# GATB/bcalm

Measured on AMD Instinct MI355X. Metric: distinct k-mers/s reads->unitigs k=31, higher is better.
Workload: dtype u64; 1 GPU; BASELINE config 3: synthetic 100000000 x 150 bp reads per GPU, k=31, abundance-min 2, 1% substitutions, 30x coverage; multi_gpu=single GPU, minimizer_size=16, log2_partitions=22

## Files before the change

bcalm_amd/csrc/devrt.h:

```cpp
#pragma once
#include <stdint.h>

#ifdef CDBG_HOSTSIM
#include "hostsim.h"
#else
#include <hip/hip_runtime.h>
#define CDBG_HD __host__ __device__ __forceinline__
#define CDBG_DEV __device__ __forceinline__
#define CDBG_SPIN_YIELD() __builtin_amdgcn_s_sleep(1)
#define CDBG_LAUNCH(kern, grid, block, stream, ...) \
    hipLaunchKernelGGL(kern, dim3((unsigned)(grid)), dim3((unsigned)(block)), 0, stream, __VA_ARGS__)
#define CDBG_SHARED __shared__
#define CDBG_WAVE_SYNC() __builtin_amdgcn_wave_barrier()
#define CDBG_PIN64(x) asm volatile("" : "+v"(x))
#endif

namespace cdbg {

CDBG_DEV uint64_t atomic_add_u64(uint64_t* p, uint64_t v) {
    return (uint64_t)atomicAdd((unsigned long long*)p, (unsigned long long)v);
}
CDBG_DEV uint64_t atomic_cas_u64(uint64_t* p, uint64_t cmp, uint64_t v) {
    return (uint64_t)atomicCAS((unsigned long long*)p, (unsigned long long)cmp, (unsigned long long)v);
}
CDBG_DEV uint64_t atomic_exch_u64(uint64_t* p, uint64_t v) {
    return (uint64_t)atomicExch((unsigned long long*)p, (unsigned long long)v);
}
#define CDBG_COMPILER_BARRIER() asm volatile("" ::: "memory")
CDBG_DEV uint64_t ld_agent_u64(const uint64_t* p) {
#ifdef CDBG_HOSTSIM
    return *p;
#else
    return __hip_atomic_load(p, __ATOMIC_RELAXED, __HIP_MEMORY_SCOPE_AGENT);
#endif
}
CDBG_DEV uint32_t ld_volatile_u32(const uint32_t* p) { return *(const volatile uint32_t*)p; }
CDBG_DEV uint32_t atomic_add_u32(uint32_t* p, uint32_t v) { return atomicAdd(p, v); }
CDBG_DEV uint32_t atomic_sub_u32(uint32_t* p, uint32_t v) { return atomicSub(p, v); }
CDBG_DEV uint32_t atomic_or_u32(uint32_t* p, uint32_t v) { return atomicOr(p, v); }
CDBG_DEV uint32_t atomic_cas_u32(uint32_t* p, uint32_t cmp, uint32_t v) { return atomicCAS(p, cmp, v); }
CDBG_DEV uint32_t atomic_max_u32(uint32_t* p, uint32_t v) { return atomicMax(p, v); }
CDBG_DEV uint32_t atomic_min_u32(uint32_t* p, uint32_t v) { return atomicMin(p, v); }
CDBG_DEV void atomic_or_u64(uint64_t* p, uint64_t v) { (void)atomicOr((unsigned long long*)p, (unsigned long long)v); }
CDBG_DEV uint64_t ld_unaligned_u64(const uint8_t* p) { uint64_t v; __builtin_memcpy(&v, p, 8); return v; }
CDBG_DEV void st_unaligned_u64(uint8_t* p, uint64_t v) { __builtin_memcpy(p, &v, 8); }
CDBG_DEV void st_unaligned_u32(uint8_t* p, uint32_t v) { __builtin_memcpy(p, &v, 4); }
CDBG_DEV void st_unaligned_u16(uint8_t* p, uint16_t v) { __builtin_memcpy(p, &v, 2); }

#ifdef CDBG_HOSTSIM
CDBG_DEV uint32_t wave_incl_sum_u32(uint32_t v) {
    const int lane = (int)(threadIdx.x & 63);
    for (int d = 1; d < 64; d <<= 1) { const uint32_t x = __shfl_up(v, (unsigned)d); if (lane >= d) v += x; }
    return v;
}
CDBG_DEV uint32_t wave_readlane_u32(uint32_t v, int src_lane) { return __shfl(v, src_lane); }
CDBG_DEV uint32_t alignbit_u32(uint32_t hi, uint32_t lo, uint32_t sh) { return (uint32_t)((((uint64_t)hi << 32) | lo) >> (sh & 31u)); }
#else
CDBG_DEV uint32_t wave_incl_sum_u32(uint32_t v) {
    v += (uint32_t)__builtin_amdgcn_update_dpp(0, (int)v, 0x111, 0xf, 0xf, false);
    v += (uint32_t)__builtin_amdgcn_update_dpp(0, (int)v, 0x112, 0xf, 0xf, false);
    v += (uint32_t)__builtin_amdgcn_update_dpp(0, (int)v, 0x114, 0xf, 0xf, false);
    v += (uint32_t)__builtin_amdgcn_update_dpp(0, (int)v, 0x118, 0xf, 0xf, false);
    v += (uint32_t)__builtin_amdgcn_update_dpp(0, (int)v, 0x142, 0xa, 0xf, false);
    v += (uint32_t)__builtin_amdgcn_update_dpp(0, (int)v, 0x143, 0xc, 0xf, false);
    return v;
}
CDBG_DEV uint32_t wave_readlane_u32(uint32_t v, int src_lane) { return (uint32_t)__builtin_amdgcn_readlane((int)v, src_lane); }
CDBG_DEV uint32_t alignbit_u32(uint32_t hi, uint32_t lo, uint32_t sh) { return __builtin_amdgcn_alignbit(hi, lo, sh); }
#endif
#ifdef CDBG_HOSTSIM
CDBG_DEV uint32_t uni_u32(uint32_t v) { return __shfl(v, 0); }
#define CDBG_NOINLINE
#define CDBG_DEV_NOINL inline
#define CDBG_LDS_BARRIER() __syncthreads()
#define CDBG_LDS_FENCE() do { } while (0)
#else
CDBG_DEV uint32_t uni_u32(uint32_t v) { return (uint32_t)__builtin_amdgcn_readfirstlane((int)v); }
#define CDBG_NOINLINE __attribute__((noinline))
#define CDBG_DEV_NOINL __device__
#define CDBG_LDS_BARRIER() do { __builtin_amdgcn_fence(__ATOMIC_RELEASE, "workgroup", "local"); __builtin_amdgcn_s_barrier(); \
                                __builtin_amdgcn_fence(__ATOMIC_ACQUIRE, "workgroup", "local"); } while (0)
#define CDBG_LDS_FENCE() __builtin_amdgcn_fence(__ATOMIC_RELEASE, "workgroup", "local")
#endif
CDBG_DEV uint64_t uni_u64(uint64_t v) { return ((uint64_t)uni_u32((uint32_t)(v >> 32)) << 32) | uni_u32((uint32_t)v); }
#ifdef CDBG_HOSTSIM
CDBG_DEV uint32_t wave_append_slots(uint32_t* cursor) { return atomic_add_u32(cursor, 1u); }
#else
CDBG_DEV uint32_t wave_append_slots(uint32_t* cursor) {
    const uint64_t act = __ballot(1);
    const uint32_t rank = __builtin_amdgcn_mbcnt_hi((uint32_t)(act >> 32), __builtin_amdgcn_mbcnt_lo((uint32_t)act, 0u));
    uint32_t base = 0;
    if (rank == 0) base = atomic_add_u32(cursor, (uint32_t)__popcll(act));
    return uni_u32(base) + rank;
}
#endif
#ifdef CDBG_HOSTSIM
CDBG_DEV uint32_t lane_pick_u32(uint64_t mask, uint32_t v, int lane) { return ((mask >> lane) & 1ULL) ? v : 0u; }
#else
CDBG_DEV uint32_t lane_pick_u32(uint64_t mask, uint32_t v, int) {
    uint32_t r;
    asm("v_cndmask_b32_e64 %0, 0, %1, %2" : "=v"(r) : "v"(v), "s"(mask));
    return r;
}
#endif
CDBG_DEV uint64_t wave_sum_u64(uint64_t v) {
#pragma unroll
    for (int d = 32; d >= 1; d >>= 1) v += __shfl_xor(v, d);
    return v;
}

}
```

bcalm_amd/csrc/k_scan.h:

```cpp
#pragma once
#include "kmer.h"

namespace cdbg {

#if defined(CDBG_PROFILE_PHASES) && !defined(CDBG_HOSTSIM)
#define CDBG_SPH(i) do { if (threadIdx.x == 0) { const uint64_t t_ = wall_clock64(); sph[i] += t_ - st_prev; st_prev = t_; } } while (0)
#else
#define CDBG_SPH(i) do { } while (0)
#endif
constexpr int SCAN_THREADS = 256;
constexpr int SCAN_GRID = 256 * 2;
constexpr int SCAN_TILE = 4096;
constexpr int SCAN_PKW = (SCAN_TILE + 16 + 256) / 16 + 11;
static_assert(SCAN_PKW % 2 == 0, "validity halves must fill whole 32-bit words");
constexpr int SCAN_NKEY = SCAN_TILE + 256;

template <int W> struct RecFmt {
    static constexpr int RW = 2 * W;
    static constexpr int CAPB = 32 * RW - 8;
};

struct ScanParams {
    const uint8_t* reads;
    uint64_t nbytes;
    uint64_t nbytes_padded;
    int k, m, log_np;
    int rank_bits, rank;
    uint32_t* part_count;
    uint64_t* part_cursor;
    uint64_t* records;
    uint64_t* stats;
    uint64_t n_tiles;
    uint32_t tile_stride, tile_offset;
    uint32_t part_cap; uint32_t* part_fill;
    uint64_t* spill_recs; uint32_t* spill_part; uint64_t* spill_cursor; uint64_t spill_cap; uint32_t* error;
    uint32_t emit_all, npl;
    const uint64_t* var_limit;
    const uint64_t* ovf;
    const uint64_t* part_off;
    uint32_t defer_slices, defer_shift, defer_nseg, defer_seg_cap;
    uint64_t defer_map;
    uint64_t* defer_recs; uint32_t* defer_part; uint32_t* defer_count;
};
constexpr int SCAN_DEFER_MAX = 16;
constexpr int SCAN_HIST = 0, SCAN_EMIT = 1, SCAN_EMIT_CAPPED = 2;
constexpr int OVF_CAP_BITS = 28;
constexpr uint64_t OVF_CAP_MASK = (1ULL << OVF_CAP_BITS) - 1ULL;

CDBG_DEV uint64_t scan_get64(const uint32_t* pk, int bitoff) {
    const int w = bitoff >> 5, sh = bitoff & 31;
    uint64_t x = ((uint64_t)pk[w] << 32) | pk[w + 1];
    return sh ? ((x << sh) | ((uint64_t)pk[w + 2] >> (32 - sh))) : x;
}
CDBG_DEV bool scan_all_valid(const uint32_t* vm, int q, int len) {
    while (len > 0) {
        const int w = q >> 5, sh = q & 31;
        uint64_t x = ((uint64_t)vm[w + 1] << 32) | vm[w];
        uint32_t bits = (uint32_t)(x >> sh);
        const int c = len < 32 ? len : 32;
        const uint32_t msk = c == 32 ? 0xFFFFFFFFu : ((1u << c) - 1u);
        if ((bits & msk) != msk) return false;
        q += c; len -= c;
    }
    return true;
}

struct alignas(16) RecPair { uint64_t lo, hi; };
#ifndef CDBG_REC16_W1
#define CDBG_REC16_W1 0
#endif
template <int MODE>
CDBG_DEV uint32_t scan_reserve_record(const ScanParams& P, uint32_t lpart) {
    if (MODE == SCAN_HIST) { atomic_add_u32(&P.part_count[lpart], 1u); return 0u; }
    return atomic_add_u32(&P.part_fill[lpart], 1u);
}
template <int W, int MODE>
CDBG_DEV uint64_t* scan_record_dst(const ScanParams& P, uint32_t lpart, uint32_t j) {
    constexpr int RW = RecFmt<W>::RW;
    if (MODE == SCAN_HIST) return nullptr;
    uint64_t* dst;
    bool fits;
    if (MODE == SCAN_EMIT) {
        uint64_t pos = (uint64_t)j;
        fits = true;
        if (P.part_off != nullptr) {
            pos += P.part_off[lpart];
            fits = P.var_limit == nullptr || pos < P.var_limit[lpart];
        }
        dst = P.records + pos * RW;
    } else {
        fits = j < P.part_cap;
        dst = P.records + ((uint64_t)lpart * P.part_cap + j) * RW;
        if (!fits && P.ovf != nullptr) {
            const uint64_t d = P.ovf[lpart];
            if ((uint64_t)j < (d & OVF_CAP_MASK)) { fits = true; dst = P.records + ((d >> OVF_CAP_BITS) + j) * RW; }
        }
    }
    if (!fits) {
        const uint64_t o = atomic_add_u64(P.spill_cursor, 1ULL);
        if (o >= P.spill_cap) { *P.error = 6; return nullptr; }
        P.spill_part[o] = lpart;
        dst = P.spill_recs + o * RW;
    }
    return dst;
}
template <int W>
CDBG_DEV void scan_store_words(uint64_t* dst, const uint64_t (&w)[RecFmt<W>::RW]) {
    constexpr int RW = RecFmt<W>::RW;
    static_assert(RW % 2 == 0, "records are pairs of words");
    if (RW == 2 && !CDBG_REC16_W1) {
        dst[1] = w[1]; CDBG_COMPILER_BARRIER(); dst[0] = w[0];
        return;
    }
#pragma unroll
    for (int i = RW - 2; i >= 0; i -= 2) {
        RecPair v; v.lo = w[i]; v.hi = w[i + 1];
        *reinterpret_cast<RecPair*>(&dst[i]) = v;
    }
}
template <int W>
CDBG_DEV void scan_record_words(const uint32_t* pk, int bitoff, uint32_t meta, uint64_t (&w)[RecFmt<W>::RW]) {
    constexpr int RW = RecFmt<W>::RW;
#pragma unroll
    for (int wv = 0; wv < RW; ++wv) {
        uint64_t x = scan_get64(pk, bitoff + 64 * wv);
        if (wv == RW - 1) x = (x & ~0xFFFFULL) | meta;
        w[RW - 1 - wv] = x;
    }
}
template <int W, int MODE>
CDBG_DEV void scan_finish_record(const ScanParams& P, const uint32_t* pk, int bitoff, uint32_t meta, uint32_t lpart, uint32_t j) {
    constexpr int RW = RecFmt<W>::RW;
    if (MODE == SCAN_HIST) return;
    uint64_t* dst = scan_record_dst<W, MODE>(P, lpart, j);
    if (dst == nullptr) return;
    if (RW == 2 && !CDBG_REC16_W1) {
#pragma unroll
        for (int wv = 0; wv < RW; ++wv) {
            uint64_t x = scan_get64(pk, bitoff + 64 * wv);
            if (wv == RW - 1) x = (x & ~0xFFFFULL) | meta;
            dst[RW - 1 - wv] = x;
        }
        return;
    }
#pragma unroll
    for (int wv = 0; wv < RW; wv += 2) {
        const uint64_t hi = scan_get64(pk, bitoff + 64 * wv);
        uint64_t lo = scan_get64(pk, bitoff + 64 * (wv + 1));
        if (wv + 1 == RW - 1) lo = (lo & ~0xFFFFULL) | meta;
        RecPair v; v.lo = lo; v.hi = hi;
        *reinterpret_cast<RecPair*>(&dst[RW - 2 - wv]) = v;
    }
}
template <int W, int MODE>
CDBG_DEV void scan_emit_record(const ScanParams& P, const uint32_t* pk, int bitoff, uint32_t meta, uint32_t lpart, uint32_t* sdefer) {
    if (MODE == SCAN_EMIT_CAPPED && P.defer_slices > 1u) {
        const uint32_t sl = (uint32_t)(P.defer_map >> (4u * (lpart >> P.defer_shift))) & 15u;
        if (sl) {
            constexpr int RW = RecFmt<W>::RW;
            uint32_t slot = P.defer_seg_cap;
            for (uint32_t q = 1; q < P.defer_slices; ++q)
                if (sl == q) slot = wave_append_slots(&sdefer[q]);
            if (slot < P.defer_seg_cap) {
                const uint64_t at = ((uint64_t)(sl - 1u) * P.defer_nseg + blockIdx.x) * P.defer_seg_cap + slot;
                uint64_t w[RW];
                scan_record_words<W>(pk, bitoff, meta, w);
                uint64_t* dst = P.defer_recs + at * RW;
#pragma unroll
                for (int i = 0; i < RW; i += 2) { RecPair v; v.lo = w[i]; v.hi = w[i + 1]; *reinterpret_cast<RecPair*>(&dst[i]) = v; }
                P.defer_part[at] = lpart;
                return;
            }
        }
    }
    scan_finish_record<W, MODE>(P, pk, bitoff, meta, lpart, scan_reserve_record<MODE>(P, lpart));
}
template <int MODE>
CDBG_DEV void scan_defer_init(const ScanParams& P, uint32_t* sdefer) { if (MODE == SCAN_EMIT_CAPPED && P.defer_slices > 1u && threadIdx.x < (unsigned)SCAN_DEFER_MAX) sdefer[threadIdx.x] = 0; }
template <int MODE>
CDBG_DEV void scan_defer_publish(const ScanParams& P, const uint32_t* sdefer) {
    if (MODE == SCAN_EMIT_CAPPED && P.defer_slices > 1u && threadIdx.x >= 1u && threadIdx.x < P.defer_slices)
        P.defer_count[(uint64_t)(threadIdx.x - 1u) * P.defer_nseg + blockIdx.x] = sdefer[threadIdx.x];
}

struct PlaceParams { ScanParams sp; uint32_t slice; };
template <int W>
__global__ void __launch_bounds__(64) k_place(PlaceParams Q) {
    constexpr int RW = RecFmt<W>::RW;
    constexpr int PLACE_U = RW <= 2 ? 4 : RW <= 4 ? 2 : 1;
    const ScanParams& P = Q.sp;
    for (uint32_t seg = blockIdx.x; seg < P.defer_nseg; seg += gridDim.x) {
        const uint64_t sidx = (uint64_t)(Q.slice - 1u) * P.defer_nseg + seg;
        const uint32_t n0 = uni_u32(P.defer_count[sidx]);
        const uint32_t n = n0 < P.defer_seg_cap ? n0 : P.defer_seg_cap;
        const uint64_t base = sidx * P.defer_seg_cap;
        for (uint32_t b = 0; b < n; b += 64u * PLACE_U) {
            uint64_t w[PLACE_U][RW]; uint32_t p[PLACE_U], j[PLACE_U];
#pragma unroll
            for (int u = 0; u < PLACE_U; ++u) {
                const uint32_t i = b + (uint32_t)u * 64u + threadIdx.x;
                p[u] = 0xFFFFFFFFu;
                if (i < n) {
                    p[u] = P.defer_part[base + i];
                    const uint64_t* src = P.defer_recs + (base + i) * RW;
#pragma unroll
                    for (int q = 0; q < RW; q += 2) { const RecPair v = *reinterpret_cast<const RecPair*>(&src[q]); w[u][q] = v.lo; w[u][q + 1] = v.hi; }
                }
            }
#pragma unroll
            for (int u = 0; u < PLACE_U; ++u) if (p[u] != 0xFFFFFFFFu) j[u] = scan_reserve_record<SCAN_EMIT_CAPPED>(P, p[u]);
#pragma unroll
            for (int u = 0; u < PLACE_U; ++u) if (p[u] != 0xFFFFFFFFu) {
                uint64_t* dst = scan_record_dst<W, SCAN_EMIT_CAPPED>(P, p[u], j[u]);
                if (dst != nullptr) scan_store_words<W>(dst, w[u]);
            }
        }
    }
}

template <int W, int MODE>
__global__ void __launch_bounds__(SCAN_THREADS) k_scan(ScanParams P) {
    constexpr int RW = RecFmt<W>::RW;
    constexpr int CAPB = RecFmt<W>::CAPB;
    CDBG_SHARED uint32_t pk[SCAN_PKW];
    CDBG_SHARED uint32_t vm[SCAN_PKW / 2 + 4];
    CDBG_SHARED uint32_t ka[SCAN_NKEY];
    CDBG_SHARED uint32_t kb[SCAN_NKEY];
    CDBG_SHARED uint64_t brk[SCAN_TILE / 64 + 2];
    CDBG_SHARED uint64_t stt[SCAN_TILE / 64 + 2];
    CDBG_SHARED uint32_t s_members, s_trav, s_nrec, s_nstart;
    CDBG_SHARED uint32_t s_defer[SCAN_DEFER_MAX];
    constexpr uint32_t LIST_CAP = (SCAN_NKEY - SCAN_TILE / 2) / 2;

    const int tid = threadIdx.x;
    const int k = P.k, m = P.m;
#if defined(CDBG_PROFILE_PHASES) && !defined(CDBG_HOSTSIM)
    uint64_t sph[8] = {0, 0, 0, 0, 0, 0, 0, 0}; uint64_t st_prev = wall_clock64();
#endif
    uint64_t n_members = 0, n_trav = 0;
    if (tid == 0) { s_members = 0; s_trav = 0; }
    scan_defer_init<MODE>(P, s_defer);
    for (uint64_t tile = blockIdx.x; tile < P.n_tiles; tile += gridDim.x) {
    const int64_t t0 = ((int64_t)tile * P.tile_stride + P.tile_offset) * SCAN_TILE;
    const int64_t base = t0 - 16;

    for (int w = tid; w < SCAN_PKW; w += SCAN_THREADS) {
        const int64_t off = base + 16 * (int64_t)w;
        uint32_t packed = 0, vbits = 0;
        if (off >= 0 && off < (int64_t)P.nbytes_padded) {
            const uint4 v = *reinterpret_cast<const uint4*>(P.reads + off);
            const uint32_t wd[4] = { v.x, v.y, v.z, v.w };
#pragma unroll
            for (int j = 0; j < 16; ++j) {
                const uint32_t c = (wd[j >> 2] >> (8 * (j & 3))) & 0xFFu;
                const uint32_t ok = ((c & 0xC0u) == 0x40u) & ((0x10008Au >> (c & 0x1Fu)) & 1u);
                packed |= base_code(c) << (30 - 2 * j);
                vbits |= ok << j;
            }
        }
        pk[w] = packed;
        reinterpret_cast<uint16_t*>(vm)[w] = (uint16_t)vbits;
    }
    if (tid < 4) vm[SCAN_PKW / 2 + tid] = 0;
    if (tid == 0) s_nrec = 0;
    __syncthreads();
    CDBG_SPH(0);

    const int WN = k - m;
    const int nkey = SCAN_TILE + WN + 1;
    for (int i = tid; i < SCAN_NKEY; i += SCAN_THREADS) {
        uint32_t key = 0xFFFFFFFFu;
        if (i < nkey) {
            const int q = 15 + i;
            if (scan_all_valid(vm, q, m)) {
                const uint64_t x = ((uint64_t)pk[q >> 4] << 32) | pk[(q >> 4) + 1];
                const uint32_t v = (uint32_t)((x << (2 * (q & 15))) >> (64 - 2 * m));
                key = mmer_key(v, m);
            }
        }
        ka[i] = key;
    }
    __syncthreads();
    CDBG_SPH(1);

    uint32_t* cur = ka; uint32_t* oth = kb;
    int width = 1;
    while (4 * width <= WN) {
        for (int i = tid; i < SCAN_NKEY; i += SCAN_THREADS) {
            uint32_t a = cur[i];
#pragma unroll
            for (int j = 1; j < 4; ++j) { const uint32_t b = (i + j * width < SCAN_NKEY) ? cur[i + j * width] : 0xFFFFFFFFu; a = a < b ? a : b; }
            oth[i] = a;
        }
        __syncthreads();
        uint32_t* t = cur; cur = oth; oth = t;
        width *= 4;
    }
    while (2 * width <= WN) {
        for (int i = tid; i < SCAN_NKEY; i += SCAN_THREADS) {
            const uint32_t a = cur[i];
            const uint32_t b = (i + width < SCAN_NKEY) ? cur[i + width] : 0xFFFFFFFFu;
            oth[i] = a < b ? a : b;
        }
        __syncthreads();
        uint32_t* t = cur; cur = oth; oth = t;
        width *= 2;
    }
    if (width != WN) {
        const int d = WN - width;
        for (int i = tid; i < SCAN_NKEY; i += SCAN_THREADS) {
            const uint32_t a = cur[i];
            const uint32_t b = (i + d < SCAN_NKEY) ? cur[i + d] : 0xFFFFFFFFu;
            oth[i] = a < b ? a : b;
        }
        __syncthreads();
        uint32_t* t = cur; cur = oth; oth = t;
    }
    const uint32_t* g = cur;
    uint32_t* lst = oth + SCAN_TILE / 2;
    CDBG_SPH(2);

    for (int it = 0; it < SCAN_TILE / SCAN_THREADS; ++it) {
        const int jq = 1 + it * SCAN_THREADS + tid;
        const unsigned long long em = __ballot(g[jq] == g[jq - 1]);
        if ((tid & 63) == 0) brk[(jq - 1) >> 6] = em;
    }
    __syncthreads();
    uint16_t* const sl = reinterpret_cast<uint16_t*>(oth);
    if (tid < 64) {
        const int K1 = k - 1, q0 = 16 + 64 * tid;
        constexpr int NXW = 5;
        uint64_t X[NXW];
#pragma unroll
        for (int j = 0; j < NXW; ++j) {
            const int bit = q0 + 64 * j, w = bit >> 5, sh = bit & 31;
            const uint64_t lo = ((uint64_t)vm[w + 1] << 32) | vm[w];
            X[j] = sh ? ((lo >> sh) | ((uint64_t)vm[w + 2] << (64 - sh))) : lo;
        }
        auto xw = [&](int i) -> uint64_t {
            uint64_t r = 0;
#pragma unroll
            for (int j = 0; j < NXW; ++j) r = (i == j) ? X[j] : r;
            return r;
        };
        auto shr_and = [&](int sft) {
            const int ws = sft >> 6, bs = sft & 63;
#pragma unroll
            for (int i = 0; i < NXW; ++i) {
                const uint64_t a0 = xw(i + ws), a1 = xw(i + ws + 1);
                X[i] &= bs ? ((a0 >> bs) | (a1 << (64 - bs))) : a0;
            }
        };
        { int len = 1; while (2 * len <= K1) { shr_and(len); len *= 2; } if (K1 > len) shr_and(K1 - len); }
        const uint64_t v = X[0];
        const uint32_t top = (uint32_t)(v >> 63);
        const uint32_t below = __shfl_up(top, 1u);
        const uint64_t vp = (v << 1) | (tid ? (uint64_t)below : 0ULL);
        uint64_t cont = v & vp & brk[tid];
        if (tid == 0) cont &= ~1ULL;
        const uint64_t starts = v & ~cont;
        brk[tid] = ~cont; stt[tid] = starts;
        const uint32_t cnt = (uint32_t)__popcll(starts);
        uint32_t off = wave_incl_sum_u32(cnt) - cnt;
        unsigned long long bits = starts;
        while (bits) { const int j = __ffsll((long long)bits) - 1; bits &= bits - 1; sl[off++] = (uint16_t)(tid * 64 + j); }
        if (tid == 63) s_nstart = off;
    }
    if (tid == 64) { brk[SCAN_TILE / 64] = ~0ULL; brk[SCAN_TILE / 64 + 1] = ~0ULL; }
    __syncthreads();
    CDBG_SPH(3);

    const int NMAX = CAPB - k + 1 < 255 ? CAPB - k + 1 : 255;
    const uint32_t rank_mask = (1u << P.rank_bits) - 1u;
    const int nstart = (int)s_nstart;
    for (int si = tid; si < nstart; si += SCAN_THREADS) {
        const int bit = sl[si];
        const int jq = bit + 1;
        const uint32_t gq = g[jq];
        const uint32_t part = part_of(gq, P.log_np);
        if (!P.emit_all && (part & rank_mask) != (uint32_t)P.rank) continue;
        const uint32_t lpart = P.emit_all ? (part & rank_mask) * P.npl + (part >> P.rank_bits) : part >> P.rank_bits;
        int e;
        {
            int nb = bit + 1;
            unsigned long long wv = brk[nb >> 6] >> (nb & 63);
            if (wv) e = nb + __ffsll((long long)wv) - 1;
            else {
                int wi = (nb >> 6) + 1;
                while (brk[wi] == 0) ++wi;
                e = wi * 64 + __ffsll((long long)brk[wi]) - 1;
            }
            if (e > SCAN_TILE) e = SCAN_TILE;
        }
        const int s = jq;
        bool first_incl = false, first_trav = false, last_incl = false, last_trav = false, first_foreign = false, last_foreign = false;
        if (scan_all_valid(vm, 15 + s - 1, k)) {
            const uint32_t g2 = g[s - 1];
            first_foreign = part_of(g2, P.log_np) != part;
            if (gq < g2) first_incl = true;
            else if (first_foreign) { first_incl = true; first_trav = true; }
        }
        if (scan_all_valid(vm, 15 + e, k)) {
            const uint32_t g2 = g[e + 1];
            last_foreign = part_of(g2, P.log_np) != part;
            if (gq < g2) last_incl = true;
            else if (last_foreign) { last_incl = true; last_trav = true; }
            else if (gq == g2) last_incl = true;
        }
        int c = s; bool firstchunk = true;
        while (c <= e) {
            const int ms = (firstchunk && first_incl) ? c - 1 : c;
            int ce = ms + NMAX - 1; if (ce > e) ce = e;
            const int me = (ce == e && !last_incl) ? e - 1 : ce;
            const int n = me - ms + 1;
            if (n > 0) {
                uint32_t meta = (uint32_t)n | (sub_of(gq, P.log_np) << 12);
                const bool ft = firstchunk && first_incl && first_trav;
                const bool lt = (ce == e) && last_incl && last_trav;
                if (ft) meta |= 0x100u;
                if (lt) meta |= 0x200u;
                if (firstchunk && first_incl && first_foreign) meta |= 0x400u;
                if ((ce == e) && last_incl && last_foreign) meta |= 0x800u;
                const uint32_t li = atomic_add_u32(&s_nrec, 1u);
                if (li < LIST_CAP) { lst[2 * li] = (uint32_t)ms | (meta << 16); lst[2 * li + 1] = lpart; }
                else scan_emit_record<W, MODE>(P, pk, 2 * (15 + ms), meta, lpart, s_defer);
                n_members += (uint64_t)n;
                n_trav += (ft ? 1 : 0) + (lt ? 1 : 0);
            }
            firstchunk = false;
            c = ce + 1;
        }
    }
    __syncthreads();
    CDBG_SPH(4);
    {
        const uint32_t nl = s_nrec < LIST_CAP ? s_nrec : LIST_CAP;
        for (uint32_t i = tid; i < nl; i += SCAN_THREADS)
            scan_emit_record<W, MODE>(P, pk, 2 * (15 + (int)(lst[2 * i] & 0xFFFFu)), lst[2 * i] >> 16, lst[2 * i + 1], s_defer);
    }
    __syncthreads();
    CDBG_SPH(5);
    }
#if defined(CDBG_PROFILE_PHASES) && !defined(CDBG_HOSTSIM)
    if (threadIdx.x == 0) for (int i = 0; i < 6; ++i) atomic_add_u64(&P.stats[16 + i], sph[i]);
#endif
    scan_defer_publish<MODE>(P, s_defer);
    if (MODE != SCAN_EMIT || P.var_limit) {
        uint32_t nm = (uint32_t)n_members, nt = (uint32_t)n_trav;
#pragma unroll
        for (int d = 32; d >= 1; d >>= 1) { nm += __shfl_xor(nm, d); nt += __shfl_xor(nt, d); }
        if ((tid & 63) == 0) { if (nm) atomic_add_u32(&s_members, nm); if (nt) atomic_add_u32(&s_trav, nt); }
        __syncthreads();
        if (tid == 0 && s_members) { atomic_add_u64(&P.stats[0], (uint64_t)s_members); atomic_add_u64(&P.stats[1], (uint64_t)s_trav); }
    }
}

constexpr int EXSCAN_THREADS = 1024;
constexpr int EXSCAN_ITEMS = 4;
constexpr int EXSCAN_BLOCK = EXSCAN_THREADS * EXSCAN_ITEMS;

CDBG_DEV uint64_t exscan_block_incl(uint64_t v, uint64_t* wsum , uint64_t& total) {
    const int tid = threadIdx.x, lane = tid & 63, wave = tid >> 6;
    uint64_t incl = v;
#pragma unroll
    for (int d = 1; d < 64; d <<= 1) { const uint64_t x = __shfl_up(incl, d); if (lane >= d) incl += x; }
    if (lane == 63) wsum[wave] = incl;
    __syncthreads();
    uint64_t basew = 0, tot = 0;
    for (int w = 0; w < EXSCAN_THREADS / 64; ++w) { const uint64_t x = wsum[w]; if (w < wave) basew += x; tot += x; }
    total = tot;
    __syncthreads();
    return incl + basew;
}
__global__ void __launch_bounds__(EXSCAN_THREADS) k_exscan_sums(const uint32_t* cnt, uint64_t* bsum, uint64_t n) {
    CDBG_SHARED uint64_t wsum[EXSCAN_THREADS / 64];
    const uint64_t i0 = (uint64_t)blockIdx.x * EXSCAN_BLOCK + (uint64_t)threadIdx.x * EXSCAN_ITEMS;
    uint64_t v = 0;
    for (int j = 0; j < EXSCAN_ITEMS; ++j) if (i0 + j < n) v += cnt[i0 + j];
    uint64_t total; exscan_block_incl(v, wsum, total);
    if (threadIdx.x == 0) bsum[blockIdx.x] = total;
}
__global__ void __launch_bounds__(EXSCAN_THREADS) k_exscan_top(uint64_t* bsum, uint64_t nb, uint64_t* off_n) {
    CDBG_SHARED uint64_t wsum[EXSCAN_THREADS / 64];
    uint64_t carry = 0;
    for (uint64_t b0 = 0; b0 < nb; b0 += EXSCAN_THREADS) {
        const uint64_t i = b0 + threadIdx.x;
        const uint64_t v = i < nb ? bsum[i] : 0;
        uint64_t total; const uint64_t incl = exscan_block_incl(v, wsum, total);
        if (i < nb) bsum[i] = carry + incl - v;
        carry += total;
    }
    if (threadIdx.x == 0) *off_n = carry;
}
__global__ void __launch_bounds__(EXSCAN_THREADS) k_exscan_apply(const uint32_t* cnt, const uint64_t* bsum, uint64_t* off, uint64_t n) {
    CDBG_SHARED uint64_t wsum[EXSCAN_THREADS / 64];
    const uint64_t i0 = (uint64_t)blockIdx.x * EXSCAN_BLOCK + (uint64_t)threadIdx.x * EXSCAN_ITEMS;
    uint32_t c[EXSCAN_ITEMS]; uint64_t v = 0;
    for (int j = 0; j < EXSCAN_ITEMS; ++j) { c[j] = (i0 + j < n) ? cnt[i0 + j] : 0u; v += c[j]; }
    uint64_t total; const uint64_t incl = exscan_block_incl(v, wsum, total);
    uint64_t acc = bsum[blockIdx.x] + incl - v;
    for (int j = 0; j < EXSCAN_ITEMS; ++j) { if (i0 + j < n) off[i0 + j] = acc; acc += c[j]; }
}
__global__ void k_max_u32(const uint32_t* a, uint64_t n, uint64_t* out) {
    uint32_t m = 0; const uint64_t stride = (uint64_t)gridDim.x * blockDim.x;
    for (uint64_t i = (uint64_t)blockIdx.x * blockDim.x + threadIdx.x; i < n; i += stride) m = a[i] > m ? a[i] : m;
#pragma unroll
    for (int d = 32; d >= 1; d >>= 1) { const uint32_t o = __shfl_xor(m, d); m = o > m ? o : m; }
    if ((threadIdx.x & 63) == 0 && m) atomic_max_u32(reinterpret_cast<uint32_t*>(out), m);
}
__global__ void k_copy_u64(const uint64_t* src, uint64_t* dst, uint64_t n) {
    const uint64_t i = (uint64_t)blockIdx.x * blockDim.x + threadIdx.x;
    if (i < n) dst[i] = src[i];
}

__global__ void k_cursor32_load(const uint64_t* off, uint32_t* cur, uint64_t n) {
    const uint64_t i = (uint64_t)blockIdx.x * blockDim.x + threadIdx.x;
    if (i < n) cur[i] = (uint32_t)off[i];
}
__global__ void k_cursor32_counts(const uint64_t* off, uint32_t* cur, uint64_t n) {
    const uint64_t i = (uint64_t)blockIdx.x * blockDim.x + threadIdx.x;
    if (i < n) cur[i] -= (uint32_t)off[i];
}

constexpr int GEN_HOSTILE = 0x100;
CDBG_HD uint32_t gen_genome_base(uint64_t gp, uint64_t G, uint64_t seed_g, bool hostile) {
    const uint32_t plain = (uint32_t)(mix64(seed_g + gp) >> 62);
    if (!hostile) return plain;
    const uint64_t hp_stride = G / 50;
    if (hp_stride >= 2400) {
        const uint64_t off = gp % hp_stride;
        if (off >= hp_stride / 2 && off < hp_stride / 2 + 600) return (uint32_t)((gp / hp_stride) & 3u);
    }
    uint64_t nc = G / 50000; if (nc > 1000) nc = 1000;
    if (nc) {
        const uint64_t rs = G / nc, off = gp % rs;
        if (off >= rs / 4 && off < rs / 4 + 5000) return (uint32_t)(mix64((seed_g ^ 0x5EED0000ULL) + (off - rs / 4)) >> 62);
    }
    const uint64_t bh = mix64(seed_g + 0x10C0000000ULL + (gp >> 12));
    if (bh % 20 == 0) {
        const uint32_t a = (uint32_t)(bh >> 8) & 3u, b2 = (a + 1u + (uint32_t)((bh >> 16) % 3)) & 3u;
        return (plain & 2u) ? a : b2;
    }
    return plain;
}
CDBG_HD uint64_t gen_read_start(uint64_t u, uint64_t G, uint64_t L, bool hostile) {
    if (hostile && (u >> 32) % 3 == 0) {
        uint64_t hot = G / 40; if (hot < L) hot = L;
        return G / 2 - hot / 2 + u % (hot - L + 1);
    }
    return u % (G - L + 1);
}
struct GenParams {
    uint8_t* out; uint64_t first_read, n_reads, total_reads, read_len; int cfg;
};
__global__ void k_gen_reads(GenParams P) {
    const uint64_t L1 = P.read_len + 1;
    const uint64_t total = P.n_reads * L1, stride = (uint64_t)gridDim.x * blockDim.x;
    const bool hostile = P.cfg >= 0 && (P.cfg & GEN_HOSTILE);
    for (uint64_t idx = (uint64_t)blockIdx.x * blockDim.x + threadIdx.x; idx < total; idx += stride) {
    const uint64_t i = idx / L1, j = idx % L1;
    if (j == P.read_len) { P.out[idx] = '\n'; continue; }
    if (P.cfg < 0) { P.out[idx] = 'A'; continue; }
    const uint64_t SEED_G = 0xBCA10000ULL + (uint64_t)P.cfg, SEED_R = 0xBCA11000ULL + (uint64_t)P.cfg,
                   SEED_E = 0xBCA12000ULL + (uint64_t)P.cfg;
    uint64_t G = (P.total_reads * P.read_len + 29) / 30;
    if (G < P.read_len) G = P.read_len;
    const uint64_t r = P.first_read + i;
    const uint64_t start = gen_read_start(mix64(SEED_R + 2 * r), G, P.read_len, hostile);
    const int strand = (int)(mix64(SEED_R + 2 * r + 1) & 1ULL);
    const uint64_t gp = strand ? start + P.read_len - 1 - j : start + j;
    uint32_t b = gen_genome_base(gp, G, SEED_G, hostile);
    if (strand) b = 3u - b;
    const uint64_t x = mix64(SEED_E + r * P.read_len + j);
    if (x % 10000 < 100) b = (b + 1 + (uint32_t)((x >> 32) % 3)) & 3u;
    P.out[idx] = (uint8_t)("ACGT"[b]);
    }
}

}
```

bcalm_amd/csrc/k_scan_fast.h:

```cpp
#pragma once
#include "k_scan.h"

namespace cdbg {

constexpr int SCANF_TILE = 4064;
constexpr int SCANF_GRID = 256 * 5;
constexpr int SCANF_WNMAX = 48;
constexpr int SCANF_NQ = 4400;
constexpr int SCANF_PKW = SCANF_NQ / 16 + 5;
CDBG_DEV int scanf_pad(int q) { return q + (q >> 4); }

CDBG_DEV uint32_t scanf_enc4(uint32_t x, uint32_t& vbits) {
    const uint32_t t = ((x >> 1) ^ (x >> 2)) & 0x03030303u;
    const uint32_t e = ((t & 0x01010101u) * 2u) + ((t & 0x02020202u) * 3u) + 0x41414141u
                     + (((t >> 1) & t & 0x01010101u) * 11u);
    const uint32_t d = e ^ (x & 0xDFDFDFDFu);
    const uint32_t z = ~((((d & 0x7F7F7F7Fu) + 0x7F7F7F7Fu) | d)) & 0x80808080u;
    vbits = (((z >> 7) * 0x01020408u) >> 24) & 0xFu;
    return (t * 0x40100401u) >> 24;
}

#ifndef CDBG_SCAN_WAVES0
#define CDBG_SCAN_WAVES0 3
#endif
#ifndef CDBG_SCAN_WAVES15
#define CDBG_SCAN_WAVES15 5
#endif
template <int W, int MODE, int WNT>
__global__ void __launch_bounds__(SCAN_THREADS, WNT == 0 ? CDBG_SCAN_WAVES0 : (WNT == 15 || WNT == 16) ? CDBG_SCAN_WAVES15 : WNT < 0 ? 2 : 4) k_scan_fast(ScanParams P) {
    constexpr int RW = RecFmt<W>::RW;
    constexpr int CAPB = RecFmt<W>::CAPB;
    CDBG_SHARED uint32_t pk2[2][SCANF_PKW];
    CDBG_SHARED uint32_t vm2[2][SCANF_PKW / 2 + 4];
    CDBG_SHARED uint32_t kg[SCANF_NQ + SCANF_NQ / 16 + 32];
    CDBG_SHARED uint32_t blk[WNT < 0 ? SCANF_NQ / 16 + 8 : 1];
    CDBG_SHARED uint32_t brk[SCANF_NQ / 32 + 4];
    CDBG_SHARED uint32_t stt[SCANF_NQ / 32 + 4];
    CDBG_SHARED uint16_t sl[SCANF_TILE + 16];
    CDBG_SHARED uint32_t s_wsum[SCAN_THREADS / 64], s_nstart, s_members, s_trav;
    CDBG_SHARED uint32_t s_defer[SCAN_DEFER_MAX];

    const int tid = threadIdx.x, lane = tid & 63, wave = tid >> 6;
    const int k = P.k, m = P.m, WN = k - m;
#if defined(CDBG_PROFILE_PHASES) && !defined(CDBG_HOSTSIM)
    uint64_t sph[8] = {0, 0, 0, 0, 0, 0, 0, 0}; uint64_t st_prev = wall_clock64();
#endif
    uint32_t n_members = 0, n_trav = 0;
    if (tid == 0) { s_members = 0; s_trav = 0; }
    scan_defer_init<MODE>(P, s_defer);
    static_assert(SCANF_PKW <= 2 * SCAN_THREADS, "two 16-byte loads per lane cover a tile");
    uint4 pv0, pv1; bool pin0 = false, pin1 = false;
    auto tile_request = [&](uint64_t tl) {
        const int64_t b = (((int64_t)tl * P.tile_stride + P.tile_offset) * SCANF_TILE) - 16;
        const int64_t o0 = b + 16 * (int64_t)tid, o1 = b + 16 * (int64_t)(tid + SCAN_THREADS);
        pin0 = o0 >= 0 && o0 < (int64_t)P.nbytes_padded;
        pin1 = tid + SCAN_THREADS < SCANF_PKW && o1 >= 0 && o1 < (int64_t)P.nbytes_padded;
        if (pin0) pv0 = *reinterpret_cast<const uint4*>(P.reads + o0);
        if (pin1) pv1 = *reinterpret_cast<const uint4*>(P.reads + o1);
    };
    auto tile_encode = [&](int buf) {
        uint32_t* const pkd = pk2[buf]; uint16_t* const vmd = reinterpret_cast<uint16_t*>(vm2[buf]);
        auto enc = [&](const uint4& v, bool in, int w) {
            uint32_t packed = 0, vbits = 0;
            if (in) {
                uint32_t v0, v1, v2, v3;
                packed = (scanf_enc4(v.x, v0) << 24) | (scanf_enc4(v.y, v1) << 16) | (scanf_enc4(v.z, v2) << 8) | scanf_enc4(v.w, v3);
                vbits = v0 | (v1 << 4) | (v2 << 8) | (v3 << 12);
            }
            pkd[w] = packed; vmd[w] = (uint16_t)vbits;
        };
        enc(pv0, pin0, tid);
        if (tid + SCAN_THREADS < SCANF_PKW) enc(pv1, pin1, tid + SCAN_THREADS);
        if (tid < 4) vm2[buf][SCANF_PKW / 2 + tid] = 0;
        if (SCANF_PKW & 1) { if (tid == 4) vmd[SCANF_PKW] = 0; }
    };
    constexpr bool PIPE = !(WNT > 32);
    int cur = 0;
    if (PIPE && (uint64_t)blockIdx.x < P.n_tiles) { tile_request(blockIdx.x); tile_encode(0); }
    if (PIPE) CDBG_LDS_BARRIER();
    for (uint64_t tile = blockIdx.x; tile < P.n_tiles; tile += gridDim.x) {
    const bool has_next = PIPE && tile + gridDim.x < P.n_tiles;
    if (has_next) tile_request(tile + gridDim.x);
    if (!PIPE) {
        const int64_t b = (((int64_t)tile * P.tile_stride + P.tile_offset) * SCANF_TILE) - 16;
        for (int w = tid; w < SCANF_PKW; w += SCAN_THREADS) {
            const int64_t off = b + 16 * (int64_t)w;
            uint32_t packed = 0, vbits = 0;
            if (off >= 0 && off < (int64_t)P.nbytes_padded) {
                const uint4 v = *reinterpret_cast<const uint4*>(P.reads + off);
                uint32_t v0, v1, v2, v3;
                packed = (scanf_enc4(v.x, v0) << 24) | (scanf_enc4(v.y, v1) << 16) | (scanf_enc4(v.z, v2) << 8) | scanf_enc4(v.w, v3);
                vbits = v0 | (v1 << 4) | (v2 << 8) | (v3 << 12);
            }
            pk2[0][w] = packed;
            reinterpret_cast<uint16_t*>(vm2[0])[w] = (uint16_t)vbits;
        }
        if (tid < 4) vm2[0][SCANF_PKW / 2 + tid] = 0;
        if (SCANF_PKW & 1) { if (tid == 4) reinterpret_cast<uint16_t*>(vm2[0])[SCANF_PKW] = 0; }
        CDBG_LDS_BARRIER();
    }
    uint32_t* const pk = pk2[cur]; uint32_t* const vm = vm2[cur];
    CDBG_SPH(0);

    const int nq_keys = 15 + SCANF_TILE + 2 + WN;
    const uint32_t mmask = m == 16 ? 0xFFFFFFFFu : ((1u << (2 * m)) - 1u);
    for (int c = tid; 16 * c < nq_keys; c += SCAN_THREADS) {
        const uint32_t w0 = pk[c], w1 = pk[c + 1];
        const uint32_t vv = (uint32_t)reinterpret_cast<const uint16_t*>(vm)[c] | ((uint32_t)reinterpret_cast<const uint16_t*>(vm)[c + 1] << 16);
        uint32_t xv = vv;
        { int len = 1; while (2 * len <= m) { xv &= xv >> len; len *= 2; } xv &= xv >> (m - len); }
        const uint64_t X = ((uint64_t)w0 << 32) | w1;
        const uint64_t RX = ~(((uint64_t)rev2_32(w1) << 32) | rev2_32(w0));
        const int fsh = 64 - 2 * m;
        uint32_t* dst = kg + 17 * c;
        uint32_t bmin = 0xFFFFFFFFu;
#pragma unroll
        for (int s = 0; s < 16; ++s) {
            const uint32_t fw = (uint32_t)(X >> (fsh - 2 * s)) & mmask;
            const uint32_t rc = (uint32_t)(RX >> (2 * s)) & mmask;
            const uint32_t key = mix32(rc < fw ? rc : fw) | (((xv >> s) & 1u) - 1u);
            dst[s] = key;
            if (WNT < 0) bmin = key < bmin ? key : bmin;
        }
        if (WNT < 0) blk[c] = bmin;
    }
    if (WNT < 0) { for (int c = (nq_keys + 15) / 16 + tid; c < SCANF_NQ / 16 + 8; c += SCAN_THREADS) blk[c] = 0xFFFFFFFFu; }
    CDBG_LDS_BARRIER();
    CDBG_SPH(1);

    uint32_t gq[16];
    const int nchunk_g = (15 + SCANF_TILE + 2 + 15) / 16;
    for (int c = tid; c < nchunk_g; c += SCAN_THREADS) {
        if (WNT < 0) {
            const int E = (WN - 1) >> 4, R = (WN - 1) & 15;
            uint32_t a[16], pe[16], pf[16];
#pragma unroll
            for (int i = 0; i < 16; ++i) { a[i] = kg[17 * c + i]; pe[i] = kg[17 * (c + E) + i]; pf[i] = kg[17 * (c + E + 1) + i]; }
            uint32_t mid = 0xFFFFFFFFu;
            for (int b = 1; b < E; ++b) { const uint32_t v = blk[c + b]; mid = v < mid ? v : mid; }
            const uint32_t full_e = blk[c + E];
#pragma unroll
            for (int i = 14; i >= 0; --i) a[i] = a[i] < a[i + 1] ? a[i] : a[i + 1];
#pragma unroll
            for (int i = 1; i < 16; ++i) { pe[i] = pe[i] < pe[i - 1] ? pe[i] : pe[i - 1]; pf[i] = pf[i] < pf[i - 1] ? pf[i] : pf[i - 1]; }
#define CDBG_TL_CASE(RR) case RR: { _Pragma("unroll") for (int j = 0; j < 16; ++j) { const int idx = j + RR; uint32_t v = a[j] < mid ? a[j] : mid;   \
                if (idx >= 16) v = v < full_e ? v : full_e;                                                                                    \
                const uint32_t tv = idx < 16 ? pe[idx < 16 ? idx : 0] : pf[idx >= 16 ? idx - 16 : 0]; gq[j] = v < tv ? v : tv; } } break;
            switch (R) { CDBG_TL_CASE(0) CDBG_TL_CASE(1) CDBG_TL_CASE(2) CDBG_TL_CASE(3) CDBG_TL_CASE(4) CDBG_TL_CASE(5) CDBG_TL_CASE(6) CDBG_TL_CASE(7)
                         CDBG_TL_CASE(8) CDBG_TL_CASE(9) CDBG_TL_CASE(10) CDBG_TL_CASE(11) CDBG_TL_CASE(12) CDBG_TL_CASE(13) CDBG_TL_CASE(14) default: CDBG_TL_CASE(15) }
#undef CDBG_TL_CASE
        } else if (WNT == 15) {
            uint32_t a[30];
#pragma unroll
            for (int i = 0; i < 30; ++i) a[i] = kg[17 * c + i + (i >> 4)];
#pragma unroll
            for (int i = 13; i >= 0; --i) a[i] = a[i] < a[i + 1] ? a[i] : a[i + 1];
#pragma unroll
            for (int i = 16; i < 30; ++i) a[i] = a[i] < a[i - 1] ? a[i] : a[i - 1];
            gq[0] = a[0]; gq[15] = a[29];
#pragma unroll
            for (int j = 1; j < 15; ++j) gq[j] = a[j] < a[j + 14] ? a[j] : a[j + 14];
        } else if (WNT == 16) {
            uint32_t a[31];
#pragma unroll
            for (int i = 0; i < 31; ++i) a[i] = kg[17 * c + i + (i >> 4)];
#pragma unroll
            for (int i = 14; i >= 0; --i) a[i] = a[i] < a[i + 1] ? a[i] : a[i + 1];
#pragma unroll
            for (int i = 17; i < 31; ++i) a[i] = a[i] < a[i - 1] ? a[i] : a[i - 1];
            gq[0] = a[0];
#pragma unroll
            for (int j = 1; j < 16; ++j) gq[j] = a[j] < a[j + 15] ? a[j] : a[j + 15];
        } else if (WNT > 0) {
            constexpr int N = 16 + WNT - 1;
            uint32_t a[N];
#pragma unroll
            for (int i = 0; i < N; ++i) a[i] = kg[scanf_pad(16 * c + i)];
            constexpr int L = WNT >= 32 ? 32 : WNT >= 16 ? 16 : WNT >= 8 ? 8 : WNT >= 4 ? 4 : WNT >= 2 ? 2 : 1;
#pragma unroll
            for (int len = 1; len < L; len *= 2) {
#pragma unroll
                for (int i = 0; i + len < N; ++i) a[i] = a[i] < a[i + len] ? a[i] : a[i + len];
            }
#pragma unroll
            for (int j = 0; j < 16; ++j) gq[j] = a[j] < a[j + WNT - L] ? a[j] : a[j + WNT - L];
        } else {
            uint32_t a[16 + SCANF_WNMAX - 1];
#pragma unroll
            for (int i = 0; i < 16 + SCANF_WNMAX - 1; ++i) a[i] = (i < 16 + WN - 1) ? kg[scanf_pad(16 * c + i)] : 0xFFFFFFFFu;
#pragma unroll
            for (int j = 0; j < 16; ++j) gq[j] = a[j];
#pragma unroll
            for (int w = 1; w < SCANF_WNMAX; ++w) {
                if (w < WN) {
#pragma unroll
                    for (int j = 0; j < 16; ++j) gq[j] = gq[j] < a[j + w] ? gq[j] : a[j + w];
                }
            }
        }
    }
    CDBG_LDS_BARRIER();
    if (tid < nchunk_g) {
#pragma unroll
        for (int j = 0; j < 16; ++j) kg[scanf_pad(16 * tid + j)] = gq[j];
    }
    CDBG_LDS_BARRIER();
    CDBG_SPH(2);
    {
        const int c = tid;
        uint32_t brk16 = 0, stt16 = 0;
        if (c >= 1 && c <= SCANF_TILE / 16) {
            const uint16_t* v16 = reinterpret_cast<const uint16_t*>(vm);
            uint32_t vj, vp;
            if (WNT < 0) {
                auto h4 = [&](int i) -> uint64_t { return (uint64_t)v16[i] | ((uint64_t)v16[i + 1] << 16) | ((uint64_t)v16[i + 2] << 32) | ((uint64_t)v16[i + 3] << 48); };
                const uint64_t w0 = h4(c - 1), w1 = h4(c + 3), w2 = h4(c + 7), w3 = (uint64_t)v16[c + 11];
                uint64_t Y[3] = { (w0 >> 15) | (w1 << 49), (w1 >> 15) | (w2 << 49), (w2 >> 15) | (w3 << 49) };
                auto yw = [&](int i) -> uint64_t { uint64_t r = 0; _Pragma("unroll") for (int j = 0; j < 3; ++j) r = (i == j) ? Y[j] : r; return r; };
                auto shr_and = [&](int sft) {
                    const int ws = sft >> 6, bs = sft & 63;
#pragma unroll
                    for (int i = 0; i < 3; ++i) { const uint64_t a0 = yw(i + ws), a1 = yw(i + ws + 1); Y[i] &= bs ? ((a0 >> bs) | (a1 << (64 - bs))) : a0; }
                };
                { const int K1 = k - 1; int len = 1; while (2 * len <= K1) { shr_and(len); len *= 2; } if (K1 > len) shr_and(K1 - len); }
                vj = (uint32_t)(Y[0] >> 1) & 0xFFFFu; vp = (uint32_t)Y[0] & 0xFFFFu;
            } else {
            const uint64_t lo = (uint64_t)v16[c - 1] | ((uint64_t)v16[c] << 16) | ((uint64_t)v16[c + 1] << 32) | ((uint64_t)v16[c + 2] << 48);
            const uint64_t hi = (uint64_t)v16[c + 3] | ((uint64_t)v16[c + 4] << 16);
            unsigned __int128 Y = (((unsigned __int128)hi << 64) | lo) >> 15;
            { const int K1 = k - 1; int len = 1; while (2 * len <= K1) { Y &= Y >> len; len *= 2; } Y &= Y >> (K1 - len); }
            vj = (uint32_t)(Y >> 1) & 0xFFFFu; vp = (uint32_t)Y & 0xFFFFu;
            }
            const uint32_t gprev = kg[scanf_pad(16 * c - 1)];
            uint32_t eq = gq[0] == gprev ? 1u : 0u;
#pragma unroll
            for (int j = 1; j < 16; ++j) eq |= (gq[j] == gq[j - 1] ? 1u : 0u) << j;
            uint32_t cont = vj & vp & eq;
            if (c == 1) cont &= ~1u;
            brk16 = ~cont & 0xFFFFu;
            stt16 = vj & ~cont;
        } else {
            brk16 = 0xFFFFu;
        }
        reinterpret_cast<uint16_t*>(brk)[c] = (uint16_t)brk16;
        reinterpret_cast<uint16_t*>(stt)[c] = (uint16_t)stt16;
        if (tid < 24) reinterpret_cast<uint16_t*>(brk)[SCAN_THREADS + tid] = 0xFFFFu;

        const int cnt = __popc(stt16);
        int incl = cnt;
#pragma unroll
        for (int d = 1; d < 64; d <<= 1) { const int x = __shfl_up(incl, d); if (lane >= d) incl += x; }
        if (lane == 63) s_wsum[wave] = (uint32_t)incl;
        CDBG_LDS_BARRIER();
        int off = incl - cnt;
        for (int w = 0; w < wave; ++w) off += (int)s_wsum[w];
        uint32_t bits = stt16;
        while (bits) { const int j = __ffs((int)bits) - 1; bits &= bits - 1; sl[off++] = (uint16_t)(16 * c + j); }
        if (tid == SCAN_THREADS - 1) s_nstart = (uint32_t)off;
    }
    CDBG_LDS_BARRIER();
    CDBG_SPH(3);

    if (has_next) tile_encode(cur ^ 1);
    const int NMAX = CAPB - k + 1;
    const uint32_t rank_mask = (1u << P.rank_bits) - 1u;
    const int nstart = (int)s_nstart;
    for (int i = tid; i < nstart; i += SCAN_THREADS) {
        const int s = sl[i];
        const uint32_t g0 = kg[scanf_pad(s)];
        const uint32_t part = part_of(g0, P.log_np);
        if (!P.emit_all && (part & rank_mask) != (uint32_t)P.rank) continue;
        const uint32_t lpart = P.emit_all ? (part & rank_mask) * P.npl + (part >> P.rank_bits) : part >> P.rank_bits;
        int e;
        {
            int nb = s + 1;
            uint32_t wv = brk[nb >> 5] >> (nb & 31);
            if (wv) e = nb + __ffs((int)wv) - 1;
            else { int wi = (nb >> 5) + 1; while (brk[wi] == 0) ++wi; e = wi * 32 + __ffs((int)brk[wi]) - 1; }
            e -= 1;
            if (e > 15 + SCANF_TILE) e = 15 + SCANF_TILE;
        }
        bool first_incl = false, first_trav = false, last_incl = false, last_trav = false, first_foreign = false, last_foreign = false;
        if (scan_all_valid(vm, s - 1, k)) {
            const uint32_t g2 = kg[scanf_pad(s - 1)];
            first_foreign = part_of(g2, P.log_np) != part;
            if (g0 < g2) first_incl = true;
            else if (first_foreign) { first_incl = true; first_trav = true; }
        }
        if (scan_all_valid(vm, e, k)) {
            const uint32_t g2 = kg[scanf_pad(e + 1)];
            last_foreign = part_of(g2, P.log_np) != part;
            if (g0 < g2) last_incl = true;
            else if (last_foreign) { last_incl = true; last_trav = true; }
            else if (g0 == g2) last_incl = true;
        }
        int c = s; bool firstchunk = true;
        while (c <= e) {
            const int ms = (firstchunk && first_incl) ? c - 1 : c;
            int ce = ms + NMAX - 1; if (ce > e) ce = e;
            const int me = (ce == e && !last_incl) ? e - 1 : ce;
            const int n = me - ms + 1;
            if (n > 0) {
                uint32_t meta = (uint32_t)n | (sub_of(g0, P.log_np) << 12);
                const bool ft = firstchunk && first_incl && first_trav;
                const bool lt = (ce == e) && last_incl && last_trav;
                if (ft) meta |= 0x100u;
                if (lt) meta |= 0x200u;
                if (firstchunk && first_incl && first_foreign) meta |= 0x400u;
                if ((ce == e) && last_incl && last_foreign) meta |= 0x800u;
                scan_emit_record<W, MODE>(P, pk, 2 * ms, meta, lpart, s_defer);
                n_members += (uint32_t)n;
                n_trav += (ft ? 1u : 0u) + (lt ? 1u : 0u);
            }
            firstchunk = false;
            c = ce + 1;
        }
    }
    CDBG_LDS_BARRIER();
    CDBG_SPH(4);
    if (PIPE) cur ^= 1;
    }
#if defined(CDBG_PROFILE_PHASES) && !defined(CDBG_HOSTSIM)
    if (threadIdx.x == 0) for (int i = 0; i < 6; ++i) atomic_add_u64(&P.stats[16 + i], sph[i]);
#endif
    scan_defer_publish<MODE>(P, s_defer);
    if (MODE != SCAN_EMIT || P.var_limit) {
#pragma unroll
        for (int d = 32; d >= 1; d >>= 1) { n_members += __shfl_xor(n_members, d); n_trav += __shfl_xor(n_trav, d); }
        if (lane == 0) { if (n_members) atomic_add_u32(&s_members, n_members); if (n_trav) atomic_add_u32(&s_trav, n_trav); }
        __syncthreads();
        if (tid == 0 && s_members) { atomic_add_u64(&P.stats[0], (uint64_t)s_members); atomic_add_u64(&P.stats[1], (uint64_t)s_trav); }
    }
}

}
```

Baseline: 24.27 billion kmers/s.

## Precompute super-k-mer boundary codes in start list and reserve record slots early

Each super-k-mer start entry in the LDS list now carries a packed boundary code for minimizer order and partition change, computed while the list is built. This replaces the per-start validity checks and extra minimizer loads in the emit loop, and the separate stt bitmap is dropped. For W==1 a new emit path reserves the output slot before assembling the record words with funnel shifts, so the atomic latency overlaps the word construction. The boundary code must fit in the spare high bits of the 16-bit entry, and the list gains a sentinel entry at its end.

Result: slower. 23.73 billion kmers/s (-2.2%).

```diff
diff --git a/bcalm_amd/csrc/devrt.h b/bcalm_amd/csrc/devrt.h
--- a/bcalm_amd/csrc/devrt.h
+++ b/bcalm_amd/csrc/devrt.h
@@ -27,6 +27,11 @@
     return (uint64_t)atomicExch((unsigned long long*)p, (unsigned long long)v);
 }
 #define CDBG_COMPILER_BARRIER() asm volatile("" ::: "memory")
+#ifdef CDBG_HOSTSIM
+#define CDBG_SETTLE_U32(x) do { } while (0)
+#else
+#define CDBG_SETTLE_U32(x) asm volatile("" : "+v"(x))
+#endif
 CDBG_DEV uint64_t ld_agent_u64(const uint64_t* p) {
 #ifdef CDBG_HOSTSIM
     return *p;
diff --git a/bcalm_amd/csrc/k_scan.h b/bcalm_amd/csrc/k_scan.h
--- a/bcalm_amd/csrc/k_scan.h
+++ b/bcalm_amd/csrc/k_scan.h
@@ -175,6 +175,66 @@
     }
     scan_finish_record<W, MODE>(P, pk, bitoff, meta, lpart, scan_reserve_record<MODE>(P, lpart));
 }
+constexpr int SCAN_BC_SHIFT = 13;
+constexpr uint32_t SCAN_BC_QMASK = (1u << SCAN_BC_SHIFT) - 1u;
+CDBG_DEV uint32_t scan_boundary_code(uint32_t gl, uint32_t gr, uint32_t valid, int log_np) {
+    const uint32_t rel = gr < gl ? 1u : gr > gl ? 2u : 3u;
+    const uint32_t f = part_of(gl, log_np) != part_of(gr, log_np) ? 1u : 0u;
+    return valid ? ((rel << 1) | f) : 0u;
+}
+CDBG_DEV uint32_t scan_first_bits(uint32_t code) {
+    const uint32_t f = code & 1u, rel = code >> 1;
+    return ((rel == 1u ? 1u : 0u) | f) | ((f && rel != 1u) ? 0x100u : 0u) | (f ? 0x400u : 0u);
+}
+CDBG_DEV uint32_t scan_last_bits(uint32_t code) {
+    const uint32_t f = code & 1u, rel = code >> 1;
+    return ((rel >= 2u ? 1u : 0u) | f) | ((f && rel != 2u) ? 0x200u : 0u) | (f ? 0x800u : 0u);
+}
+CDBG_DEV uint32_t scan_funnel(uint32_t a, uint32_t b, int sh) { return (uint32_t)((((((uint64_t)a) << 32) | b) << sh) >> 32); }
+template <int W>
+CDBG_DEV void scan_record_words_seq(const uint32_t* pk, int bitoff, uint32_t meta, uint64_t (&w)[RecFmt<W>::RW]) {
+    constexpr int RW = RecFmt<W>::RW;
+    const int w0 = bitoff >> 5, sh = bitoff & 31;
+    uint32_t d[2 * RW + 1];
+#pragma unroll
+    for (int i = 0; i < 2 * RW + 1; ++i) d[i] = pk[w0 + i];
+#pragma unroll
+    for (int wv = 0; wv < RW; ++wv) {
+        uint64_t x = ((uint64_t)scan_funnel(d[2 * wv], d[2 * wv + 1], sh) << 32) | scan_funnel(d[2 * wv + 1], d[2 * wv + 2], sh);
+        if (wv == RW - 1) x = (x & ~0xFFFFULL) | meta;
+        w[RW - 1 - wv] = x;
+    }
+}
+template <int W, int MODE>
+CDBG_DEV void scan_emit_record_early(const ScanParams& P, const uint32_t* pk, int bitoff, uint32_t meta, uint32_t lpart, uint32_t* sdefer) {
+    constexpr int RW = RecFmt<W>::RW;
+    if (MODE == SCAN_HIST) { scan_reserve_record<MODE>(P, lpart); return; }
+    uint32_t dsl = 0, slot = 0;
+    if (MODE == SCAN_EMIT_CAPPED && P.defer_slices > 1u) {
+        dsl = (uint32_t)(P.defer_map >> (4u * (lpart >> P.defer_shift))) & 15u;
+        if (dsl) {
+            slot = P.defer_seg_cap;
+            for (uint32_t q = 1; q < P.defer_slices; ++q)
+                if (dsl == q) slot = wave_append_slots(&sdefer[q]);
+            if (slot >= P.defer_seg_cap) dsl = 0;
+        }
+    }
+    uint32_t j = 0;
+    if (!dsl) j = scan_reserve_record<MODE>(P, lpart);
+    uint64_t w[RW];
+    scan_record_words_seq<W>(pk, bitoff, meta, w);
+    CDBG_SETTLE_U32(j);
+    if (dsl) {
+        const uint64_t at = ((uint64_t)(dsl - 1u) * P.defer_nseg + blockIdx.x) * P.defer_seg_cap + slot;
+        uint64_t* dst = P.defer_recs + at * RW;
+#pragma unroll
+        for (int i = 0; i < RW; i += 2) { RecPair v; v.lo = w[i]; v.hi = w[i + 1]; *reinterpret_cast<RecPair*>(&dst[i]) = v; }
+        P.defer_part[at] = lpart;
+        return;
+    }
+    uint64_t* dst = scan_record_dst<W, MODE>(P, lpart, j);
+    if (dst != nullptr) scan_store_words<W>(dst, w);
+}
 template <int MODE>
 CDBG_DEV void scan_defer_init(const ScanParams& P, uint32_t* sdefer) { if (MODE == SCAN_EMIT_CAPPED && P.defer_slices > 1u && threadIdx.x < (unsigned)SCAN_DEFER_MAX) sdefer[threadIdx.x] = 0; }
 template <int MODE>
diff --git a/bcalm_amd/csrc/k_scan_fast.h b/bcalm_amd/csrc/k_scan_fast.h
--- a/bcalm_amd/csrc/k_scan_fast.h
+++ b/bcalm_amd/csrc/k_scan_fast.h
@@ -26,6 +26,9 @@
 #ifndef CDBG_SCAN_WAVES15
 #define CDBG_SCAN_WAVES15 5
 #endif
+#ifndef CDBG_SCAN_RESERVE_FIRST
+#define CDBG_SCAN_RESERVE_FIRST 1
+#endif
 template <int W, int MODE, int WNT>
 __global__ void __launch_bounds__(SCAN_THREADS, WNT == 0 ? CDBG_SCAN_WAVES0 : (WNT == 15 || WNT == 16) ? CDBG_SCAN_WAVES15 : WNT < 0 ? 2 : 4) k_scan_fast(ScanParams P) {
     constexpr int RW = RecFmt<W>::RW;
@@ -35,7 +38,6 @@
     CDBG_SHARED uint32_t kg[SCANF_NQ + SCANF_NQ / 16 + 32];
     CDBG_SHARED uint32_t blk[WNT < 0 ? SCANF_NQ / 16 + 8 : 1];
     CDBG_SHARED uint32_t brk[SCANF_NQ / 32 + 4];
-    CDBG_SHARED uint32_t stt[SCANF_NQ / 32 + 4];
     CDBG_SHARED uint16_t sl[SCANF_TILE + 16];
     CDBG_SHARED uint32_t s_wsum[SCAN_THREADS / 64], s_nstart, s_members, s_trav;
     CDBG_SHARED uint32_t s_defer[SCAN_DEFER_MAX];
@@ -208,8 +210,8 @@
     CDBG_SPH(2);
     {
         const int c = tid;
-        uint32_t brk16 = 0, stt16 = 0;
-        if (c >= 1 && c <= SCANF_TILE / 16) {
+        uint32_t brk16 = 0, stt16 = 0, vk = 0;
+        if (c >= 1 && c <= SCANF_TILE / 16 + 1) {
             const uint16_t* v16 = reinterpret_cast<const uint16_t*>(vm);
             uint32_t vj, vp;
             if (WNT < 0) {
@@ -231,19 +233,18 @@
             { const int K1 = k - 1; int len = 1; while (2 * len <= K1) { Y &= Y >> len; len *= 2; } Y &= Y >> (K1 - len); }
             vj = (uint32_t)(Y >> 1) & 0xFFFFu; vp = (uint32_t)Y & 0xFFFFu;
             }
+            vk = vj & vp;
             const uint32_t gprev = kg[scanf_pad(16 * c - 1)];
             uint32_t eq = gq[0] == gprev ? 1u : 0u;
 #pragma unroll
             for (int j = 1; j < 16; ++j) eq |= (gq[j] == gq[j - 1] ? 1u : 0u) << j;
-            uint32_t cont = vj & vp & eq;
+            uint32_t cont = vk & eq;
             if (c == 1) cont &= ~1u;
             brk16 = ~cont & 0xFFFFu;
             stt16 = vj & ~cont;
-        } else {
-            brk16 = 0xFFFFu;
-        }
+        }
+        if (c < 1 || c > SCANF_TILE / 16) { brk16 = 0xFFFFu; stt16 = 0; }
         reinterpret_cast<uint16_t*>(brk)[c] = (uint16_t)brk16;
-        reinterpret_cast<uint16_t*>(stt)[c] = (uint16_t)stt16;
         if (tid < 24) reinterpret_cast<uint16_t*>(brk)[SCAN_THREADS + tid] = 0xFFFFu;
 
         const int cnt = __popc(stt16);
@@ -255,8 +256,16 @@
         int off = incl - cnt;
         for (int w = 0; w < wave; ++w) off += (int)s_wsum[w];
         uint32_t bits = stt16;
-        while (bits) { const int j = __ffs((int)bits) - 1; bits &= bits - 1; sl[off++] = (uint16_t)(16 * c + j); }
-        if (tid == SCAN_THREADS - 1) s_nstart = (uint32_t)off;
+        while (bits) {
+            const int j = __ffs((int)bits) - 1; bits &= bits - 1;
+            const int q = 16 * c + j;
+            sl[off++] = (uint16_t)((uint32_t)q | (scan_boundary_code(kg[scanf_pad(q - 1)], kg[scanf_pad(q)], (vk >> j) & 1u, P.log_np) << SCAN_BC_SHIFT));
+        }
+        if (tid == SCAN_THREADS - 1) {
+            const int q = 16 + SCANF_TILE;
+            sl[off] = (uint16_t)((uint32_t)q | (scan_boundary_code(kg[scanf_pad(q - 1)], gq[0], vk & 1u, P.log_np) << SCAN_BC_SHIFT));
+            s_nstart = (uint32_t)off;
+        }
     }
     CDBG_LDS_BARRIER();
     CDBG_SPH(3);
@@ -266,7 +275,8 @@
     const uint32_t rank_mask = (1u << P.rank_bits) - 1u;
     const int nstart = (int)s_nstart;
     for (int i = tid; i < nstart; i += SCAN_THREADS) {
-        const int s = sl[i];
+        const uint32_t sl0 = sl[i], sl1 = sl[i + 1];
+        const int s = (int)(sl0 & SCAN_BC_QMASK);
         const uint32_t g0 = kg[scanf_pad(s)];
         const uint32_t part = part_of(g0, P.log_np);
         if (!P.emit_all && (part & rank_mask) != (uint32_t)P.rank) continue;
@@ -280,20 +290,10 @@
             e -= 1;
             if (e > 15 + SCANF_TILE) e = 15 + SCANF_TILE;
         }
-        bool first_incl = false, first_trav = false, last_incl = false, last_trav = false, first_foreign = false, last_foreign = false;
-        if (scan_all_valid(vm, s - 1, k)) {
-            const uint32_t g2 = kg[scanf_pad(s - 1)];
-            first_foreign = part_of(g2, P.log_np) != part;
-            if (g0 < g2) first_incl = true;
-            else if (first_foreign) { first_incl = true; first_trav = true; }
-        }
-        if (scan_all_valid(vm, e, k)) {
-            const uint32_t g2 = kg[scanf_pad(e + 1)];
-            last_foreign = part_of(g2, P.log_np) != part;
-            if (g0 < g2) last_incl = true;
-            else if (last_foreign) { last_incl = true; last_trav = true; }
-            else if (g0 == g2) last_incl = true;
-        }
+        const uint32_t fb = scan_first_bits(sl0 >> SCAN_BC_SHIFT);
+        const uint32_t lb = scan_last_bits((int)(sl1 & SCAN_BC_QMASK) == e + 1 ? sl1 >> SCAN_BC_SHIFT : 0u);
+        const bool first_incl = fb & 1u, last_incl = lb & 1u;
+        const uint32_t meta0 = sub_of(g0, P.log_np) << 12;
         int c = s; bool firstchunk = true;
         while (c <= e) {
             const int ms = (firstchunk && first_incl) ? c - 1 : c;
@@ -301,16 +301,13 @@
             const int me = (ce == e && !last_incl) ? e - 1 : ce;
             const int n = me - ms + 1;
             if (n > 0) {
-                uint32_t meta = (uint32_t)n | (sub_of(g0, P.log_np) << 12);
-                const bool ft = firstchunk && first_incl && first_trav;
-                const bool lt = (ce == e) && last_incl && last_trav;
-                if (ft) meta |= 0x100u;
-                if (lt) meta |= 0x200u;
-                if (firstchunk && first_incl && first_foreign) meta |= 0x400u;
-                if ((ce == e) && last_incl && last_foreign) meta |= 0x800u;
-                scan_emit_record<W, MODE>(P, pk, 2 * ms, meta, lpart, s_defer);
+                uint32_t meta = (uint32_t)n | meta0;
+                if (firstchunk) meta |= fb & 0x500u;
+                if (ce == e) meta |= lb & 0xA00u;
+                if (CDBG_SCAN_RESERVE_FIRST && W == 1) scan_emit_record_early<W, MODE>(P, pk, 2 * ms, meta, lpart, s_defer);
+                else scan_emit_record<W, MODE>(P, pk, 2 * ms, meta, lpart, s_defer);
                 n_members += (uint32_t)n;
-                n_trav += (ft ? 1u : 0u) + (lt ? 1u : 0u);
+                n_trav += ((meta >> 8) & 1u) + ((meta >> 9) & 1u);
             }
             firstchunk = false;
             c = ce + 1;
```
